# qgallouedec/deep_rl

Hardware: AMD Instinct MI355X
Metric: env-steps/sec + updates/sec, PPO CartPole-v1 4096 envs/GPU (higher is better)
Workload: dtype f32

## Files before the change

### deep_rl_amd/csrc/mi_grad_kernel.inc

```
struct __attribute__((aligned(16))) GV(grad_weights) {
#if GRAD_BX
    bf16x8 W2g[4 * 2 * 3 * 64];
    bf16x8 W2t[4 * 2 * 3 * 64];
#else
    float W2g[HID * HID];
    float W2t[HID * HID];
#endif
    float b1[HID], b2[HID];
    float W3[2 * HID];
    float W1s[HID * OBS];
    float b3s[4];
#if GRAD_BX
    union { unsigned short imgH[BX_IMG]; float bufB[TROWS * W2S]; } hb[GRAD_WAVES];
    unsigned short imgZ[GRAD_WAVES][BX_IMG];
    float xs[GRAD_WAVES][TROWS * 4];
#else
    float bufA[GRAD_WAVES][TROWS * W2S];
    float bufB[GRAD_WAVES][TROWS * W2S];
    float bufC[GRAD_WAVES][TROWS * W2S];
#endif
};
struct __attribute__((aligned(16))) GV(grad_smem) {
    union {
        GV(grad_weights) w;
        float red[GRAD_WAVES][RED_STRIDE];
    };
    double nrm[4];
    double nparts[256];
};
#if GRAD_BX
#define XS(row, k) xs[(row) * 4 + (k)]
#else
#define XS(row, k) bufA[(row) * W2S + HID + (k)]
#endif

template <bool ACTOR>
__device__ __forceinline__ void GV(grad_body)(GV(grad_smem)& sm, const float* __restrict__ params, const grad_pending_t& pend,
                                          const float* __restrict__ observations,
                                          const int64_t* __restrict__ actions, const float* __restrict__ log_probs,
                                          const float* __restrict__ advantages, const float* __restrict__ returns,
                                          const float* __restrict__ values, const int32_t* __restrict__ idx, int mb,
                                          const double* __restrict__ adv_sums, float clip_coef, float ent_coef, float vf_coef,
                                          float invn, float* __restrict__ part, unsigned vb, grad_role_t rl) {
    constexpr int NOUT = ACTOR ? 2 : 1;
    constexpr int BASE = ACTOR ? 0 : C_BASE;
    constexpr bool ANTI = ACTOR;
    constexpr int NHEAD = ANTI ? 1 : NOUT;
    const int tid = threadIdx.x, lane = tid & 63, wib = tid >> 6;
    const int j = lane & 15, g = lane >> 4;
    const bool pending = pend.grads != nullptr;
    const float* p = (pending ? pend.p_in : params) + BASE;
    GV(grad_weights)& W = sm.w;
#ifdef GRAD_STAMPS
    unsigned long long rt_in, rt_ready, rt_loop;
    asm volatile("s_memrealtime %0\n\ts_waitcnt lgkmcnt(0)" : "=s"(rt_in) :: "memory");
#endif

#ifdef GRAD_STAMPS
    unsigned long long pro_t[6] = {0, 0, 0, 0, 0, 0};
    asm volatile("s_memtime %0\n\ts_waitcnt lgkmcnt(0)" : "=s"(pro_t[0]) :: "memory");
#endif
    {
        const int q = (tid >> 4) & 15, cg = tid & 15;
        const bool writer = pending && rl.ri == 0;
        const bool w2t = tid < 256;
        constexpr int NT_A = N_W2, NT_B = HID + NOUT * HID;
        const bool has0 = tid < NT_A + NT_B, has1 = tid < NOUT;
        const int f0 = !has0 ? 0 : (tid < NT_A ? tid : N_B2 + (tid - NT_A));
        const int f1 = N_W3 + NOUT * HID + (has1 ? tid : 0);
        f32x4 w[4];
#pragma unroll
        for (int e = 0; e < 4; ++e) w[e] = w2t ? reinterpret_cast<const f32x4*>(p + N_W2)[(4 * q + e) * 16 + cg] : f32x4{0.0f, 0.0f, 0.0f, 0.0f};
        float sp0 = p[f0], sp1 = p[f1];
        if (pending) {
            f32x4 gg[4], mm[4], vv[4];
#pragma unroll
            for (int e = 0; e < 4; ++e) {
                const int at = w2t ? (4 * q + e) * 16 + cg : 0;
                gg[e] = reinterpret_cast<const f32x4*>(pend.grads + BASE + N_W2)[at];
                mm[e] = reinterpret_cast<const f32x4*>(pend.m_in + BASE + N_W2)[at];
                vv[e] = reinterpret_cast<const f32x4*>(pend.v_in + BASE + N_W2)[at];
            }
            const float sg0 = pend.grads[BASE + f0], sg1 = pend.grads[BASE + f1];
            float sm0 = pend.m_in[BASE + f0], sv0 = pend.v_in[BASE + f0], sm1 = pend.m_in[BASE + f1], sv1 = pend.v_in[BASE + f1];
            const bool hold = __hip_atomic_load(pend.gate, __ATOMIC_RELAXED, __HIP_MEMORY_SCOPE_AGENT) != 0u;
            const float a_w1 = hold ? 0.0f : pend.w1, a_b2 = hold ? 1.0f : pend.b2, a_w2 = hold ? 0.0f : pend.w2, a_ss = hold ? 0.0f : pend.step_size;
#ifdef GRAD_STAMPS
            asm volatile("s_memtime %0\n\ts_waitcnt lgkmcnt(0)" : "=s"(pro_t[1]) :: "memory");
#endif
            const float total = block_grad_norm(pend.grads, pend.norm_parts, NPARAMS, sm.nrm, sm.nparts);
#ifdef GRAD_STAMPS
            asm volatile("s_memtime %0\n\ts_waitcnt lgkmcnt(0)" : "=s"(pro_t[2]) :: "memory");
#endif
            float coef = pend.max_norm / (total + 1e-6f);
            coef = coef > 1.0f ? 1.0f : coef;
            if (pend.grad_norm && vb == 0 && tid == 0) *pend.grad_norm = total;
            if (w2t) {
#pragma unroll
                for (int e = 0; e < 4; ++e) {
#pragma unroll
                    for (int x = 0; x < 4; ++x) {
// ... 37 lines not shown
                unsigned h0, m0, l0, h1_, m1, l1;
                split3(w[0][x], w[1][x], h0, m0, l0); split3(w[2][x], w[3][x], h1_, m1, l1);
                const int lane_a = (i & 15) + 16 * (q & 3), slot = 4 * ((q >> 2) & 1);
                const int base = (((i >> 4) * 2 + (q >> 3)) * 3) * 64 * 8 + lane_a * 8 + slot;
                *reinterpret_cast<uint2*>(timg + base) = make_uint2(h0, h1_);
                *reinterpret_cast<uint2*>(timg + base + 64 * 8) = make_uint2(m0, m1);
                *reinterpret_cast<uint2*>(timg + base + 2 * 64 * 8) = make_uint2(l0, l1);
            }
#else
#pragma unroll
            for (int e = 0; e < 4; ++e) *reinterpret_cast<f32x4*>(&W.W2g[(cg * 64 + 4 * q + e) * 4]) = w[e] * GRAD_PS;
#pragma unroll
            for (int x = 0; x < 4; ++x) *reinterpret_cast<f32x4*>(&W.W2t[(q * 64 + 4 * cg + x) * 4]) = f32x4{w[0][x], w[1][x], w[2][x], w[3][x]};
#endif
        }
        if (has0) {
            if (tid < N_B1) W.W1s[tid] = GRAD_PS * sp0;
            else if (tid < NT_A) W.b1[tid - N_B1] = GRAD_PS * sp0;
            else if (tid < NT_A + HID) W.b2[tid - NT_A] = GRAD_PS * sp0;
            else W.W3[tid - NT_A - HID] = sp0;
        }
        if (has1) W.b3s[tid] = sp1;
    }

    float adv_mean = 0.0f, adv_rden = 1.0f;
    if constexpr (ACTOR) {
        const double s1 = adv_sums[0], s2 = adv_sums[1], cnt = adv_sums[2];
        const double mean = s1 / cnt;
        double var = (s2 - s1 * mean) / (cnt - 1.0);
        var = var < 0.0 ? 0.0 : var;
        adv_mean = (float)mean;
        adv_rden = 1.0f / ((float)sqrt(var) + 1e-8f);
    }

    const int n_tiles = (mb + TROWS - 1) / TROWS;
    const int half = rl.nr * 4;
    const bool split_ok = (gridDim.x % (2u << GRAD_ROLE_BIT)) == 0;
    const bool young = split_ok && wib >= 4;
    const int wi_half = rl.ri * 4 + (wib & 3);
    int tile, stride, tile_end;
    if (split_ok) {
        const int rounds = (n_tiles + half - 1) / half;
        const int old_rounds = (rounds * GRAD_OLD_SHARE + 8) / 16;
        const int split = old_rounds * half < n_tiles ? old_rounds * half : n_tiles;
        const int wi = wi_half;
        stride = half;
        tile = young ? split + wi : wi;
        tile_end = young ? n_tiles : split;
    } else {
        stride = rl.nr * GRAD_WAVES;
        tile = rl.ri * GRAD_WAVES + wib;
        tile_end = n_tiles;
    }
    auto tile_rid = [&](int t) { const int row = t * TROWS + j; return idx[row < mb ? row : mb - 1]; };
    int rid_next = tile_rid(tile + stride);
    row_in cur = gather_row<ACTOR>(tile_rid(tile), g, observations, actions, log_probs, advantages, returns, values);
#ifdef GRAD_STAMPS
    asm volatile("s_memtime %0\n\ts_waitcnt lgkmcnt(0)" : "=s"(pro_t[4]) :: "memory");
#endif
    __syncthreads();
    float w1f[4], b3[NOUT];
#pragma unroll
    for (int mt = 0; mt < 4; ++mt) w1f[mt] = W.W1s[4 * (16 * mt + j) + g];
#pragma unroll
    for (int a = 0; a < NOUT; ++a) b3[a] = W.b3s[a];
    f32x4 w3d[4];
    if constexpr (ANTI) {
#pragma unroll
        for (int mt = 0; mt < 4; ++mt) {
            const float4 w0 = *reinterpret_cast<const float4*>(&W.W3[16 * mt + 4 * g]), w1 = *reinterpret_cast<const float4*>(&W.W3[HID + 16 * mt + 4 * g]);
            w3d[mt] = f32x4{w0.x - w1.x, w0.y - w1.y, w0.z - w1.z, w0.w - w1.w};
        }
    }
#ifdef GRAD_STAMPS
    asm volatile("s_memtime %0\n\ts_waitcnt lgkmcnt(0)" : "=s"(pro_t[5]) :: "memory");
#endif

#if GRAD_BX
    f32x16 dW2x[2][2];
#pragma unroll
    for (int ot = 0; ot < 2; ++ot)
#pragma unroll
        for (int it2 = 0; it2 < 2; ++it2)
#pragma unroll
            for (int q = 0; q < 16; ++q) dW2x[ot][it2][q] = 0.0f;
    f32x4 db2v[4];
#pragma unroll
    for (int mt = 0; mt < 4; ++mt) db2v[mt] = f32x4{0.0f, 0.0f, 0.0f, 0.0f};
#else
    f32x4 dW2[4][4];
#pragma unroll
    for (int mo = 0; mo < 4; ++mo)
#pragma unroll
        for (int mi = 0; mi < 4; ++mi) dW2[mo][mi] = f32x4{0.0f, 0.0f, 0.0f, 0.0f};
#endif
    f32x4 dW1a = {0.0f, 0.0f, 0.0f, 0.0f}, dW1b = dW1a;
    f32x4 dW3v[NHEAD][4];
#pragma unroll
    for (int a = 0; a < NHEAD; ++a)
#pragma unroll
        for (int mt = 0; mt < 4; ++mt) dW3v[a][mt] = f32x4{0.0f, 0.0f, 0.0f, 0.0f};
    float db1 = 0.0f, db3[2] = {0.0f, 0.0f};
#if !GRAD_BX
    float db2[4] = {0.0f, 0.0f, 0.0f, 0.0f};
#endif
    float loss_a = 0.0f, loss_b = 0.0f;

#if GRAD_BX
    unsigned short* imgH = W.hb[wib].imgH;
    unsigned short* imgZ = W.imgZ[wib];
    float* bufB = W.hb[wib].bufB;
    float* xs = W.xs[wib];
#else
    float* bufA = W.bufA[wib];
    float* bufB = W.bufB[wib];
    float* bufC = W.bufC[wib];
#endif

#ifdef GRAD_STAMPS
    asm volatile("s_memrealtime %0\n\ts_waitcnt lgkmcnt(0)" : "=s"(rt_ready) :: "memory");
    unsigned long long stamp_acc[12] = {0, 0, 0, 0, 0, 0, 0, 0, 0, 0, 0, 0}, stamp_last, stamp_t0;
    asm volatile("s_memtime %0\n\ts_waitcnt lgkmcnt(0)" : "=s"(stamp_last) :: "memory");
    stamp_t0 = stamp_last;
#endif
    int it = 0;
    for (; tile < tile_end; tile += stride, ++it) {
        const bool valid = tile * TROWS + j < mb;
        const row_in nxt = gather_row<ACTOR>(rid_next, g, observations, actions, log_probs, advantages, returns, values);
        rid_next = tile_rid(tile + 2 * stride);

        XS(j, g) = cur.x;
        STAMP(0);

        f32x4 h1[4];
#pragma unroll
        for (int mt = 0; mt < 4; ++mt) {
            const float4 b = *reinterpret_cast<const float4*>(&W.b1[16 * mt + 4 * g]);
            h1[mt] = mfma16(w1f[mt], cur.x, f32x4{b.x, b.y, b.z, b.w});
        }
#pragma unroll
        for (int mt = 0; mt < 4; ++mt)
#pragma unroll
            for (int r = 0; r < 4; ++r) h1[mt][r] = GRAD_TANH(h1[mt][r]);
#if !GRAD_BX
#pragma unroll
        for (int mt = 0; mt < 4; ++mt) *reinterpret_cast<float4*>(bufA + j * W2S + 16 * mt + 4 * g) = make_float4(h1[mt][0], h1[mt][1], h1[mt][2], h1[mt][3]);
#endif
        STAMP(1);

        f32x4 h2[4];
#pragma unroll
        for (int mt = 0; mt < 4; ++mt) {
            const float4 b = *reinterpret_cast<const float4*>(&W.b2[16 * mt + 4 * g]);
            h2[mt] = f32x4{b.x, b.y, b.z, b.w};
        }
#if GRAD_BX
        wave_lds_fence();
#pragma unroll
        for (int sh = 0; sh < 2; ++sh) {
            const bx_parts bq = split8(h1[2 * sh], h1[2 * sh + 1]);
            bx_store_image(imgH, bq, sh, g, j);
#pragma unroll
            for (int mt = 0; mt < 4; ++mt) {
                bf16x8 a[3];
#pragma unroll
                for (int pp = 0; pp < 3; ++pp) a[pp] = W.W2g[((mt * 2 + sh) * 3 + pp) * 64 + lane];
                h2[mt] = bx_mac(a, bq, h2[mt]);
            }
        }
#else
#pragma unroll
        for (int c = 0; c < 4; ++c) {
            f32x4 a[4];
#pragma unroll
            for (int mt = 0; mt < 4; ++mt) a[mt] = *reinterpret_cast<const f32x4*>(&W.W2g[((4 * c + g) * 64 + 16 * mt + j) * 4]);
#pragma unroll
            for (int r = 0; r < 4; ++r)
#pragma unroll
                for (int mt = 0; mt < 4; ++mt) h2[mt] = mfma16(a[mt][r], h1[c][r], h2[mt]);
        }
#endif
        STAMP(2);
#pragma unroll
        for (int mt = 0; mt < 4; ++mt)
// ... 111 lines not shown
        for (int sh = 0; sh < 2; ++sh) {
            const bx_parts bq = split8(dz2[2 * sh], dz2[2 * sh + 1]);
            bx_store_image(imgZ, bq, sh, g, j);
#pragma unroll
            for (int mt = 0; mt < 4; ++mt) {
                bf16x8 a[3];
#pragma unroll
                for (int pp = 0; pp < 3; ++pp) a[pp] = W.W2t[((mt * 2 + sh) * 3 + pp) * 64 + lane];
                dz1[mt] = bx_mac(a, bq, dz1[mt]);
            }
        }
#pragma unroll
        for (int mt = 0; mt < 4; ++mt) db2v[mt] += dz2[mt];
        wave_lds_fence();
        {
            const int at = (lane >> 5) * BX_HALF + (lane & 31) * 8;
#pragma unroll
            for (int it2 = 0; it2 < 2; ++it2) {
                bf16x8 hbv[3];
#pragma unroll
                for (int pp = 0; pp < 3; ++pp) hbv[pp] = *reinterpret_cast<const bf16x8*>(imgH + pp * BX_PART + 32 * it2 * 8 + at);
#pragma unroll
                for (int ot = 0; ot < 2; ++ot) {
                    bf16x8 za[3];
#pragma unroll
                    for (int pp = 0; pp < 3; ++pp) za[pp] = *reinterpret_cast<const bf16x8*>(imgZ + pp * BX_PART + 32 * ot * 8 + at);
                    dW2x[ot][it2] = bx_mac32(za, hbv, dW2x[ot][it2]);
                }
            }
        }
#else
#pragma unroll
        for (int c = 0; c < 4; ++c) {
            f32x4 a[4];
#pragma unroll
            for (int mt = 0; mt < 4; ++mt) a[mt] = *reinterpret_cast<const f32x4*>(&W.W2t[((4 * c + g) * 64 + 16 * mt + j) * 4]);
#pragma unroll
            for (int r = 0; r < 4; ++r)
#pragma unroll
                for (int mt = 0; mt < 4; ++mt) dz1[mt] = mfma16(a[mt][r], dz2[c][r], dz1[mt]);
        }
#endif
#pragma unroll
        for (int mt = 0; mt < 4; ++mt)
#pragma unroll
            for (int r = 0; r < 4; ++r) { const float t = h1[mt][r]; dz1[mt][r] = dz1[mt][r] * __builtin_fmaf(-t, t, 1.0f); }

        STAMP(7);
        wave_lds_fence();
#pragma unroll
        for (int mt = 0; mt < 4; ++mt)
            *reinterpret_cast<float4*>(bufB + j * W2S + 16 * mt + 4 * g) = make_float4(dz1[mt][0], dz1[mt][1], dz1[mt][2], dz1[mt][3]);
        wave_lds_fence();
#pragma unroll
        for (int rr = 0; rr < TROWS; rr += 2) {
            const float z0 = bufB[rr * W2S + lane], z1v = bufB[(rr + 1) * W2S + lane];
            db1 += z0 + z1v;
            dW1a = mfma4(z0, XS(rr, lane & 3), dW1a);
            dW1b = mfma4(z1v, XS(rr + 1, lane & 3), dW1b);
        }

        STAMP(8);
#if !GRAD_BX
        wave_lds_fence();
#pragma unroll
        for (int s = 0; s < 4; ++s) {
            const int ro = (s + 4 * g) * W2S + j;
            float a[4], b[4];
#pragma unroll
            for (int m = 0; m < 4; ++m) { a[m] = bufC[ro + 16 * m]; b[m] = bufA[ro + 16 * m]; db2[m] += a[m]; }
#pragma unroll
            for (int mo = 0; mo < 4; ++mo)
#pragma unroll
                for (int mi = 0; mi < 4; ++mi) dW2[mo][mi] = mfma16(a[mo], b[mi], dW2[mo][mi]);
        }
#endif
        STAMP(9);
        cur = nxt;
        STAMP(10);
    }
#ifdef GRAD_STAMPS
    if (lane == 0) {
        unsigned long long* dbg = STAMP_BASE(part) + 32 * wib;
        unsigned long long now;
        asm volatile("s_memtime %0\n\ts_waitcnt lgkmcnt(0)" : "=s"(now) :: "memory");
        for (int k = 0; k < 11; ++k) dbg[k] = stamp_acc[k];
        dbg[11] = now - stamp_t0;
        dbg[12] = (unsigned long long)it;
        for (int k = 0; k < 6; ++k) dbg[20 + k] = pro_t[k];
    }
    asm volatile("s_memrealtime %0\n\ts_waitcnt lgkmcnt(0)" : "=s"(rt_loop) :: "memory");
#endif
    const f32x4 dW1 = dW1a + dW1b;

    __syncthreads();
    {
        float* slot = sm.red[wib];
#if GRAD_BX
#pragma unroll
        for (int ot = 0; ot < 2; ++ot)
#pragma unroll
            for (int it2 = 0; it2 < 2; ++it2)
#pragma unroll
                for (int qq = 0; qq < 4; ++qq) {
                    const int o = 32 * ot + 8 * qq + 4 * (lane >> 5), i = 32 * it2 + (lane & 31);
                    const f32x16& d = dW2x[ot][it2];
                    *reinterpret_cast<f32x4*>(&slot[((4 * (o >> 4) + (i >> 4)) * 64 + (i & 15) + 16 * ((o & 15) >> 2)) * 4]) =
                        f32x4{d[4 * qq], d[4 * qq + 1], d[4 * qq + 2], d[4 * qq + 3]};
                }
#else
#pragma unroll
        for (int mo = 0; mo < 4; ++mo)
#pragma unroll
            for (int mi = 0; mi < 4; ++mi) *reinterpret_cast<f32x4*>(&slot[((4 * mo + mi) * 64 + lane) * 4]) = dW2[mo][mi];
#endif
        float* sm_small = slot + HID * HID;
#pragma unroll
        for (int i = 0; i < 4; ++i) sm_small[(4 * (lane >> 2) + i) * 4 + (lane & 3)] = dW1[i];
        sm_small[256 + lane] = db1;
#if GRAD_BX
#pragma unroll
        for (int mt = 0; mt < 4; ++mt)
#pragma unroll
            for (int r = 0; r < 4; ++r) {
                float t = db2v[mt][r];
                t += dpp_xor1(t); t += dpp_xor2(t); t += dpp_half_mirror(t); t += dpp_mirror(t);
                if (j == 0) sm_small[320 + 16 * mt + 4 * g + r] = t;
            }
#else
#pragma unroll
        for (int m = 0; m < 4; ++m) {
            const float t = groups_sum(db2[m]);
// ... 26 lines not shown
    for (int k = 0; k < HID * HID / 4 / (64 * GRAD_WAVES); ++k) {
        const int i = tid + 64 * GRAD_WAVES * k;
        const f32x4 a0 = reinterpret_cast<const f32x4*>(sm.red[0])[i], a1 = reinterpret_cast<const f32x4*>(sm.red[1])[i];
        const f32x4 a2 = reinterpret_cast<const f32x4*>(sm.red[2])[i], a3 = reinterpret_cast<const f32x4*>(sm.red[3])[i];
        const f32x4 a4 = reinterpret_cast<const f32x4*>(sm.red[4])[i], a5 = reinterpret_cast<const f32x4*>(sm.red[5])[i];
        const f32x4 a6 = reinterpret_cast<const f32x4*>(sm.red[6])[i], a7 = reinterpret_cast<const f32x4*>(sm.red[7])[i];
        reinterpret_cast<f32x4*>(part + N_W2)[i] = ((a0 + a2) + (a1 + a3)) + ((a4 + a6) + (a5 + a7));
    }
    constexpr int N_SMALL = 384 + NOUT * HID + NOUT;
    for (int i = tid; i < 522; i += 64 * GRAD_WAVES) {
        if (i >= N_SMALL && i < 520) continue;
        float t = (sm.red[0][HID * HID + i] + sm.red[1][HID * HID + i]) + (sm.red[2][HID * HID + i] + sm.red[3][HID * HID + i]);
        t += (sm.red[4][HID * HID + i] + sm.red[5][HID * HID + i]) + (sm.red[6][HID * HID + i] + sm.red[7][HID * HID + i]);
        int dst;
        if (i < 256) dst = N_W1 + i;
        else if (i < 320) dst = N_B1 + (i - 256);
        else if (i < 384) dst = N_B2 + (i - 320);
        else if (i < N_SMALL) dst = N_W3 + (i - 384);
        else dst = PART_LOSS + (i - 520);
        part[dst] = t;
    }
#ifdef GRAD_STAMPS
    if (lane == 0) {
        unsigned long long rt_out;
        asm volatile("s_memrealtime %0\n\ts_waitcnt lgkmcnt(0)" : "=s"(rt_out) :: "memory");
        unsigned long long* dbg = STAMP_BASE(part) + 32 * wib;
        dbg[13] = rt_in; dbg[14] = rt_ready; dbg[15] = rt_loop; dbg[16] = rt_out;
        const unsigned hw_id = __builtin_amdgcn_s_getreg((31 << 11) | 4), xcc = __builtin_amdgcn_s_getreg((31 << 11) | 20);
        dbg[17] = ((unsigned long long)xcc << 32) | hw_id;
    }
#endif
}

__global__ void __launch_bounds__(64 * GRAD_WAVES, GRAD_WPS)
GV(grad_kernel)(const float* __restrict__ params, grad_pending_t pend, const float* __restrict__ observations, const int64_t* __restrict__ actions,
            const float* __restrict__ log_probs, const float* __restrict__ advantages, const float* __restrict__ returns,
            const float* __restrict__ values, const int32_t* __restrict__ idx, int mb, const double* __restrict__ adv_sums,
            float clip_coef, float ent_coef, float vf_coef, float invn, float* __restrict__ workspace) {
    __shared__ GV(grad_smem) sm;
    MI_INSIDE_SCOPE(MI_PROF_GRAD);
    const unsigned rb = GRAD_ROLE_BIT;
    const unsigned lowmask = (1u << rb) - 1u;
    const unsigned vb = (gridDim.x & ((2u << rb) - 1u)) ? blockIdx.x
                                                        : ((blockIdx.x >> rb) & 1u) | (((blockIdx.x & lowmask) | ((blockIdx.x >> (rb + 1)) << rb)) << 1);
    float* part = workspace + (size_t)vb * PART_STRIDE;
    const grad_role_t rl = grad_role(vb, (int)gridDim.x);
    if (rl.role == 0)
        GV(grad_body)<true>(sm, params, pend, observations, actions, log_probs, advantages, returns, values, idx, mb, adv_sums, clip_coef,
                        ent_coef, vf_coef, invn, part, vb, rl);
    else
        GV(grad_body)<false>(sm, params, pend, observations, actions, log_probs, advantages, returns, values, idx, mb, adv_sums, clip_coef,
                         ent_coef, vf_coef, invn, part, vb, rl);
}

#undef XS
```

### deep_rl_amd/csrc/mi_update.hip

```cpp
#include "mi_common.h"

typedef float f32x16 __attribute__((ext_vector_type(16)));
typedef float f32x4 __attribute__((ext_vector_type(4)));

__global__ void __launch_bounds__(64) gae_kernel(const float* __restrict__ rewards, const float* __restrict__ dones,
                                                 const float* __restrict__ values, int T, int N, float gamma, float lam,
                                                 float* __restrict__ adv, float* __restrict__ returns) {
    const int i = blockIdx.x * blockDim.x + threadIdx.x;
    if (i >= N) return;
    float last = 0.0f;
    float vnext = values[(size_t)T * N + i];
    adv[(size_t)T * N + i] = 0.0f;
    returns[(size_t)T * N + i] = 0.0f + vnext;
#pragma unroll 8
    for (int t = T - 1; t >= 0; --t) {
        const size_t c = (size_t)t * N + i, n = c + N;
        const float vcur = values[c];
        const float a = gamma * (1.0f - dones[n]);
        const float b = vnext + lam * last;
        float v = rewards[n] + a * b;
        v = v - vcur;
        adv[c] = v;
        returns[c] = v + vcur;
        last = v;
// ... 258 lines not shown
        }
        if ((lane & 15) == 0) {
            const int row = lane >> 4, k0 = (row & 1) + 9 * (row >> 1);
#pragma unroll
            for (int q = 0; q < 4; ++q) sparts[w + 8 * (2 * q + k0)] = s[q];
            if ((row & 1) == 0) sparts[w + 8 * (8 + 9 * (row >> 1))] = s[4];
        }
        __syncthreads();
        if (t < 256) S = sparts[t];
    } else {
        const bool perm = n == NPARAMS;
        if (t < 256) sparts[t] = 0.0;
        __syncthreads();
        constexpr int U = 6;
        for (int b0 = w; b0 < nb; b0 += nw * U) {
            float x[U];
#pragma unroll
            for (int u = 0; u < U; ++u) {
                const int b = b0 + nw * u, p = 64 * b + lane;
                x[u] = (b < nb && p < n) ? grads[perm ? ppo_slab_to_param(p) : p] : 0.0f;
            }
#pragma unroll
            for (int u = 0; u < U; ++u) {
                const int b = b0 + nw * u;
                const double sb = wave_butterfly_f64((double)x[u] * (double)x[u]);
                if (lane == 0 && b < nb) sparts[b & 255] = sparts[b & 255] + sb;
            }
        }
        __syncthreads();
        if (t < 256) S = sparts[t];
    }
    S = wave_butterfly_f64(S);
    if (t < 256 && lane == 0) ws[w] = S;
    __syncthreads();
    return (float)sqrt((ws[0] + ws[1]) + (ws[2] + ws[3]));
}

struct grad_pending_t {
    const float* grads;
    const float* p_in; const float* m_in; const float* v_in;
    float* p_out; float* m_out; float* v_out;
    float* grad_norm;
    const double* norm_parts;
    const uint32_t* gate;
    float w1, b2, w2, step_size, rbc2, eps, max_norm;
};

struct grad_role_t { int role, ri, nr; };
__host__ __device__ inline grad_role_t grad_role(unsigned vb, int n_blocks) {
    return grad_role_t{(int)(vb & 1u), (int)(vb >> 1), n_blocks >> 1};
}
__host__ __device__ inline int grad_slab(int role, int ri) { return 2 * ri + role; }

struct row_in {
    float x;
    int act;
    float f0, f1;
};

template <bool ACTOR>
__device__ __forceinline__ row_in gather_row(int rid, int g, const float* __restrict__ observations, const int64_t* __restrict__ actions,
                                             const float* __restrict__ log_probs, const float* __restrict__ advantages,
                                             const float* __restrict__ returns, const float* __restrict__ values) {
    row_in r;
    r.x = observations[4 * (size_t)rid + g];
    if constexpr (ACTOR) {
        r.act = reinterpret_cast<const int*>(actions)[2 * (size_t)rid];
        r.f0 = log_probs[rid]; r.f1 = advantages[rid];
    } else {
        r.act = 0;
        r.f0 = returns[rid]; r.f1 = values[rid];
    }
    return r;
}

#ifdef GRAD_STAMPS
#define STAMP(k) do { __builtin_amdgcn_sched_barrier(0); { unsigned long long t_; asm volatile("s_memtime %0\n\ts_waitcnt lgkmcnt(0)" : "=s"(t_) :: "memory"); \
                      stamp_acc[k] += t_ - stamp_last; stamp_last = t_; } __builtin_amdgcn_sched_barrier(0); } while (0)
#define STAMP_BASE(part) (reinterpret_cast<unsigned long long*>((part) + (size_t)(GRAD_MAX_BLOCKS / 2) * PART_STRIDE))
#else
#define STAMP(k) do {} while (0)
#endif

#define GRAD_BX 0
#define GV(x) x##_f32
#include "mi_grad_kernel.inc"
#undef GRAD_BX
#undef GV
#define GRAD_BX 1
#define GV(x) x##_bx
#include "mi_grad_kernel.inc"
#undef GRAD_BX
#undef GV

#define RED_PARAMS 64
#define RED_GROUPS 16
template <int WORLD>
__global__ void __launch_bounds__(RED_PARAMS * RED_GROUPS)
grad_reduce_kernel(const float* __restrict__ workspace, int n_blocks, float ent_coef, float vf_coef, double inv_count,
                   float* __restrict__ grads, float* __restrict__ loss_terms, double* __restrict__ norm_parts, const p2p_args_t x) {
    MI_INSIDE_SCOPE(MI_PROF_REDUCE);
    const int pblocks = (NPARAMS + RED_PARAMS - 1) / RED_PARAMS;
    if ((int)blockIdx.x < pblocks) {
        __shared__ float part[RED_GROUPS][RED_PARAMS];
        const int pl = threadIdx.x & (RED_PARAMS - 1), sg = threadIdx.x >> 6;
        const int p = blockIdx.x * RED_PARAMS + pl;
        float acc = 0.0f;
        const int role = p < C_BASE ? 0 : 1;
        const int off = p - (role ? C_BASE : 0);
        if (p < NPARAMS) {
            const float* src = workspace + off;
            const int nr = n_blocks >> 1;
            if (nr <= 9 * RED_GROUPS) {
                float v[9];
#pragma unroll
                for (int u = 0; u < 9; ++u) { const int k = sg + RED_GROUPS * u; v[u] = k < nr ? src[(size_t)grad_slab(role, k) * PART_STRIDE] : 0.0f; }
#pragma unroll
                for (int u = 0; u < 9; ++u) if (sg + RED_GROUPS * u < nr) acc += v[u];
            } else {
#pragma unroll 4
                for (int k = sg; k < nr; k += RED_GROUPS) acc += src[(size_t)grad_slab(role, k) * PART_STRIDE];
            }
        }
        part[sg][pl] = acc;
// ... 97 lines not shown
                           const float* advantages, const float* returns, const float* values, const int32_t* idx, int mb, const double* adv_sums,
                           float clip_coef, float ent_coef, float vf_coef, double inv_count, void* workspace, float* grads, float* loss_terms,
                           hipStream_t s, void* p2p = nullptr) {
    int blocks = grad_blocks();
    const int tiles = (mb + TROWS - 1) / TROWS;
    const int need = 2 * ((tiles + GRAD_WAVES - 1) / GRAD_WAVES);
    if (need < blocks) blocks = need;
    {
        mi_prof_scope prof(MI_PROF_GRAD, s);
        if (g_contraction == MI_CONTRACTION_BF16X3)
            grad_kernel_bx<<<blocks, 64 * GRAD_WAVES, 0, s>>>(params, pend, observations, actions, log_probs, advantages, returns, values, idx, mb,
                                                              adv_sums, clip_coef, ent_coef, vf_coef, (float)inv_count, (float*)workspace);
        else
            grad_kernel_f32<<<blocks, 64 * GRAD_WAVES, 0, s>>>(params, pend, observations, actions, log_probs, advantages, returns, values, idx, mb,
                                                               adv_sums, clip_coef, ent_coef, vf_coef, (float)inv_count, (float*)workspace);
    }
    MI_LAUNCH_CHECK();
    {
        mi_prof_scope prof(MI_PROF_REDUCE, s);
        static_assert((NPARAMS + RED_PARAMS - 1) / RED_PARAMS == NORM_BLOCKS && RED_PARAMS == 64, "one norm block per reduction workgroup");
        p2p_args_t x;
        memset(&x, 0, sizeof(x));
        int world = 0;
        if (p2p) {
            if (loss_terms != grads + NPARAMS) { mi_set_error("ppo_grad_launch: the P2P exchange needs loss_terms == grads + MI_PPO_NPARAMS"); return MI_EINVAL; }
            int rc = mi_comm_p2p_next(p2p, (size_t)NPARAMS + 4, &x, &world, s);
            if (rc) return rc;
        }
        const float* ws = (const float*)workspace;
        double* np = ws_norm_parts(workspace);
        switch (world) {
            case 0: grad_reduce_launch<0>(s, ws, blocks, ent_coef, vf_coef, inv_count, grads, loss_terms, np, x); break;
            case 1: grad_reduce_launch<1>(s, ws, blocks, ent_coef, vf_coef, inv_count, grads, loss_terms, np, x); break;
            case 2: grad_reduce_launch<2>(s, ws, blocks, ent_coef, vf_coef, inv_count, grads, loss_terms, np, x); break;
            case 3: grad_reduce_launch<3>(s, ws, blocks, ent_coef, vf_coef, inv_count, grads, loss_terms, np, x); break;
            case 4: grad_reduce_launch<4>(s, ws, blocks, ent_coef, vf_coef, inv_count, grads, loss_terms, np, x); break;
            case 5: grad_reduce_launch<5>(s, ws, blocks, ent_coef, vf_coef, inv_count, grads, loss_terms, np, x); break;
            case 6: grad_reduce_launch<6>(s, ws, blocks, ent_coef, vf_coef, inv_count, grads, loss_terms, np, x); break;
            case 7: grad_reduce_launch<7>(s, ws, blocks, ent_coef, vf_coef, inv_count, grads, loss_terms, np, x); break;
            default: grad_reduce_launch<8>(s, ws, blocks, ent_coef, vf_coef, inv_count, grads, loss_terms, np, x); break;
        }
    }
    MI_LAUNCH_CHECK();
    return MI_OK;
}

extern "C" int mi_ppo_minibatch_grad(const float* params, const float* observations, const int64_t* actions,
                                     const float* log_probs, const float* advantages, const float* returns,
                                     const float* values, const int32_t* idx, int mb, const double* adv_sums, float clip_coef,
                                     float ent_coef, float vf_coef, double inv_count, void* workspace, float* grads,
                                     float* loss_terms, void* stream) {
    MI_CHECK_ARG(params && observations && actions && log_probs && advantages && returns && values && idx && adv_sums, "NULL input");
    MI_CHECK_ARG(workspace && grads, "NULL workspace/grads");
    MI_CHECK_ARG(mb > 0, "mb must be positive");
    return ppo_grad_launch(params, no_pending(), observations, actions, log_probs, advantages, returns, values, idx, mb, adv_sums, clip_coef, ent_coef,
                           vf_coef, inv_count, workspace, grads, loss_terms, (hipStream_t)stream);
}

__global__ void __launch_bounds__(512) clip_adam_kernel(const float* p_in, const float* m_in, const float* v_in, float* p_out, float* m_out, float* v_out,
                                                         const float* __restrict__ grads, int n, float w1, float b2,
                                                         float w2, float step_size, float rbc2, float eps, float max_norm,
                                                         float* __restrict__ grad_norm, const double* __restrict__ norm_parts, const uint32_t* __restrict__ gate) {
    __shared__ double ws[4], sparts[256];
    MI_INSIDE_SCOPE(MI_PROF_CLIP_ADAM);
    const bool hold = mi_gate_closed(gate);
    const int i = blockIdx.x * blockDim.x + threadIdx.x;
    const bool live = i < n;
    float pm = live ? m_in[i] : 0.0f, pv = live ? v_in[i] : 0.0f;
    const float pp = live ? p_in[i] : 0.0f, pg = live ? grads[i] : 0.0f;
    const float total = block_grad_norm(grads, norm_parts, n, ws, sparts);
    float coef = max_norm / (total + 1e-6f);
    coef = coef > 1.0f ? 1.0f : coef;
    if (grad_norm && blockIdx.x == 0 && threadIdx.x == 0) *grad_norm = total;
    if (live) {
        float np = pp;
        if (!hold) np = mi_adam_elem(pp, pg * coef, pm, pv, w1, b2, w2, step_size, rbc2, eps);
        m_out[i] = pm; v_out[i] = pv;
        p_out[i] = np;
    }
}

struct adam_consts_t { float w1, b2, w2, step_size, rbc2, eps; };
static adam_consts_t adam_consts(int64_t step, double lr, double beta1, double beta2, double eps) {
    const double bc1 = 1.0 - pow(beta1, (double)step), bc2 = 1.0 - pow(beta2, (double)step);
    adam_consts_t k;
    k.w1 = (float)(1.0 - beta1); k.b2 = (float)beta2; k.w2 = (float)(1.0 - beta2);
    k.step_size = (float)(lr / bc1); k.rbc2 = (float)(1.0 / sqrt(bc2)); k.eps = (float)eps;
    return k;
}

static int clip_adam_launch(const float* p_in, const float* m_in, const float* v_in, float* p_out, float* m_out, float* v_out, const float* grads, int n,
                            const adam_consts_t& k, float max_norm, float* grad_norm, const double* norm_parts, hipStream_t s, const uint32_t* gate = nullptr) {
    mi_prof_scope prof(MI_PROF_CLIP_ADAM, s);
    const int threads = n == NPARAMS ? 512 : 256;
    clip_adam_kernel<<<(n + threads - 1) / threads, threads, 0, s>>>(p_in, m_in, v_in, p_out, m_out, v_out, grads, n, k.w1, k.b2, k.w2, k.step_size, k.rbc2, k.eps, max_norm,
                                                                    grad_norm, norm_parts, gate);
    MI_LAUNCH_CHECK();
    return MI_OK;
}

int mi_clip_adam_gated(float* params, const float* grads, float* exp_avg, float* exp_avg_sq, int n, int64_t step, double lr, double beta1, double beta2, double eps,
                       float max_norm, float* grad_norm, void* comm, void* stream) {
    return clip_adam_launch(params, exp_avg, exp_avg_sq, params, exp_avg, exp_avg_sq, grads, n, adam_consts(step, lr, beta1, beta2, eps), max_norm, grad_norm,
                            nullptr, (hipStream_t)stream, mi_comm_gate(comm));
}

extern "C" int mi_clip_adam(float* params, const float* grads, float* exp_avg, float* exp_avg_sq, int n, int64_t step, double lr,
                            double beta1, double beta2, double eps, float max_norm, float* grad_norm, void* stream) {
// ... 70 lines not shown
    hipStream_t s = (hipStream_t)stream;
    const int mb = n_rows / n_minibatch;
    if (mb % PS_PER_BLOCK == 0 && epochs <= PS_MAX_EPOCHS) {
        MI_HIP(hipMemsetAsync(sums_all, 0, sizeof(double) * 3 * (size_t)n_minibatch * epochs, s));
        ps_epochs_t pe;
        for (int ep = 0; ep < epochs; ++ep) {
            const uint64_t key = mi_perm_key(seed, (uint64_t)update_index, (uint64_t)ep);
            pe.k0[ep] = (uint32_t)key; pe.k1[ep] = (uint32_t)(key >> 32); pe.out[ep] = perm_all + (size_t)ep * n_rows;
        }
        uint32_t bits = 1;
        while ((1u << bits) < (uint32_t)n_rows) ++bits;
        if (bits < 2) bits = 2;
        mi_prof_scope prof(MI_PROF_STATS, s);
        perm_stats_kernel<<<dim3((n_rows + PS_PER_BLOCK - 1) / PS_PER_BLOCK, epochs), 256, 0, s>>>((uint32_t)n_rows, bits / 2, bits - bits / 2, pe, mb, n_minibatch, advantages,
                                                                                                 sums_all);
        MI_LAUNCH_CHECK();
        return MI_OK;
    }
    for (int ep = 0; ep < epochs; ++ep) {
        int rc = mi_make_perm((uint32_t)n_rows, mi_perm_key(seed, (uint64_t)update_index, (uint64_t)ep), perm_all + (size_t)ep * n_rows, stream);
        if (rc) return rc;
        rc = mi_adv_stats(advantages, perm_all + (size_t)ep * n_rows, mb, n_minibatch, sums_all + (size_t)3 * n_minibatch * ep, stream);
        if (rc) return rc;
    }
    return MI_OK;
}

struct opt_set_t { float* p; float* m; float* v; };

static int ppo_update_impl(void* handle, const mi_ppo_buffers_t* b, const mi_ppo_hparams_t* hp, void* comm, int world, void* stream);

extern "C" int mi_ppo_update(void* handle, const mi_ppo_buffers_t* b, const mi_ppo_hparams_t* hp, void* stream) {
    return ppo_update_impl(handle, b, hp, nullptr, 1, stream);
}

extern "C" int mi_ppo_update_sharded(void* handle, const mi_ppo_buffers_t* b, const mi_ppo_hparams_t* hp, void* comm, void* stream) {
    int world = 1;
    if (comm) {
        int rc = mi_comm_poll_impl(comm);
        if (rc) return rc;
        rc = mi_comm_info(comm, &world, nullptr, nullptr, nullptr);
        if (rc) return rc;
        MI_CHECK_ARG(b && b->loss_terms == b->grads + NPARAMS, "sharded update: loss_terms must be grads + MI_PPO_NPARAMS (one buffer, one all-reduce)");
    }
    return ppo_update_impl(handle, b, hp, comm, world, stream);
}

static int ppo_update_impl(void* handle, const mi_ppo_buffers_t* b, const mi_ppo_hparams_t* hp, void* comm, int world, void* stream) {
    MI_CHECK_ARG(handle && b && hp, "NULL pointer");
    MI_CHECK_ARG(hp->T > 0 && hp->n_minibatch > 0 && hp->update_epochs > 0, "bad hyper-parameters");
    mi_env* e = (mi_env*)handle;
    const int N = e->n, B = hp->T * N;
    MI_CHECK_ARG(B % hp->n_minibatch == 0, "T*N must be divisible by n_minibatch");
    const int mb = B / hp->n_minibatch;
    const bool fused = (mb % PS_PER_BLOCK) == 0;
    const bool p2p = comm != nullptr && mi_comm_p2p_fused_ok(comm);
    const bool sharded_norm = (world > 1 && !p2p) || g_assume_sharded != 0;
    int rc = mi_rollout_gae_internal(handle, b->params, hp->T, b->obs_cur, b->observations, b->values, b->actions, b->log_probs, b->rewards,
                                     b->dones, b->episodes, b->episode_stats, b->max_ep, hp->gamma, hp->gae_lambda, b->advantages, b->returns,
                                     fused ? b->adv_sums : nullptr, 3 * hp->n_minibatch * hp->update_epochs, b->episode_stats_next, stream);
    if (rc) return rc;
    hipStream_t s = (hipStream_t)stream;
    if (fused && hp->update_epochs <= PS_MAX_EPOCHS) {
        ps_epochs_t pe;
        for (int ep = 0; ep < hp->update_epochs; ++ep) {
            const uint64_t key = mi_perm_key(e->seed, (uint64_t)hp->update_index, (uint64_t)ep);
            pe.k0[ep] = (uint32_t)key; pe.k1[ep] = (uint32_t)(key >> 32); pe.out[ep] = b->perm + (size_t)ep * B;
        }
        uint32_t bits = 1;
        while ((1u << bits) < (uint32_t)B) ++bits;
        if (bits < 2) bits = 2;
        mi_prof_scope prof(MI_PROF_STATS, s);
        perm_stats_kernel<<<dim3((B + PS_PER_BLOCK - 1) / PS_PER_BLOCK, hp->update_epochs), 256, 0, s>>>((uint32_t)B, bits / 2, bits - bits / 2, pe, mb, hp->n_minibatch,
                                                                                                       b->advantages, b->adv_sums);
        MI_LAUNCH_CHECK();
    } else {
        rc = mi_ppo_perms_and_stats(e->seed, hp->update_index, hp->update_epochs, B, hp->n_minibatch, b->advantages, b->perm, b->adv_sums, stream);
        if (rc) return rc;
    }
    if (comm) {
        mi_prof_scope prof(MI_PROF_COMM_STATS, s);
        rc = mi_comm_allreduce_impl(comm, b->adv_sums, (size_t)3 * hp->n_minibatch * hp->update_epochs, 1, s);
        if (rc) return rc;
    }
    float* spare = reinterpret_cast<float*>(b->workspace) + (size_t)(GRAD_MAX_BLOCKS - GRAD_SPARE_SLABS) * PART_STRIDE;
    const opt_set_t caller = {b->params, b->exp_avg, b->exp_avg_sq};
    const opt_set_t sets[2] = {{spare, spare + STATE_STRIDE, spare + 2 * STATE_STRIDE},
                               {spare + 3 * STATE_STRIDE, spare + 4 * STATE_STRIDE, spare + 5 * STATE_STRIDE}};
    opt_set_t cur = caller;
    int64_t step = hp->opt_step;
    bool owed = false;
    int flip = 0;
    for (int ep = 0; ep < hp->update_epochs; ++ep) {
        const double* sums = b->adv_sums + (size_t)3 * hp->n_minibatch * ep;
        const int32_t* perm = b->perm + (size_t)ep * B;
        for (int k = 0; k < hp->n_minibatch; ++k) {
            grad_pending_t pend = no_pending();
            if (owed) {
                const adam_consts_t c = adam_consts(step, hp->lr, hp->beta1, hp->beta2, hp->eps);
                const opt_set_t out = sets[flip];
                flip ^= 1;
                pend.grads = b->grads; pend.p_in = cur.p; pend.m_in = cur.m; pend.v_in = cur.v; pend.p_out = out.p; pend.m_out = out.m; pend.v_out = out.v;
                pend.grad_norm = b->grad_norm; pend.w1 = c.w1; pend.b2 = c.b2; pend.w2 = c.w2; pend.step_size = c.step_size; pend.rbc2 = c.rbc2; pend.eps = c.eps;
                pend.max_norm = hp->max_grad_norm;
                pend.norm_parts = sharded_norm ? nullptr : ws_norm_parts(b->workspace);
                pend.gate = ppo_gate(comm);
// ... 209 lines not shown
```

Measured before the change: 396.3 million.

## Split grad loop into full and ragged tiles, use 32-bit gathers and LDS bases

Restructures the gradient kernel's tile loop so that full tiles run without bounds clamping and at most one ragged tail tile runs separately. Global gathers now use 32-bit byte offsets with scalar bases instead of 64-bit indexing, and the wave index is made uniform via readfirstlane. Per-wave LDS buffers are regrouped into one struct, LDS read pointers are hoisted out of the loop, and the x values are read back as vector loads. The aim is less address arithmetic and fewer VGPRs in the hot loop, paid for by a new 2^28-row limit on storage and extra code size.

```diff
diff --git a/deep_rl_amd/csrc/mi_grad_kernel.inc b/deep_rl_amd/csrc/mi_grad_kernel.inc
--- a/deep_rl_amd/csrc/mi_grad_kernel.inc
+++ b/deep_rl_amd/csrc/mi_grad_kernel.inc
@@ -10,16 +10,19 @@
     float W3[2 * HID];
     float W1s[HID * OBS];
     float b3s[4];
-#if GRAD_BX
-    union { unsigned short imgH[BX_IMG]; float bufB[TROWS * W2S]; } hb[GRAD_WAVES];
-    unsigned short imgZ[GRAD_WAVES][BX_IMG];
-    float xs[GRAD_WAVES][TROWS * 4];
-#else
-    float bufA[GRAD_WAVES][TROWS * W2S];
-    float bufB[GRAD_WAVES][TROWS * W2S];
-    float bufC[GRAD_WAVES][TROWS * W2S];
-#endif
+    struct {
+#if GRAD_BX
+        union { unsigned short imgH[BX_IMG]; float bufB[TROWS * W2S]; } hb;
+        unsigned short imgZ[BX_IMG];
+#else
+        float bufA[TROWS * W2S];
+        float bufB[TROWS * W2S];
+        float bufC[TROWS * W2S];
+#endif
+        float xs[4 * TROWS];
+    } __attribute__((aligned(16))) st[GRAD_WAVES];
 };
+static_assert(TROWS == 16, "xs is read back as four b128 per lane");
 struct __attribute__((aligned(16))) GV(grad_smem) {
     union {
         GV(grad_weights) w;
@@ -28,11 +31,6 @@
     double nrm[4];
     double nparts[256];
 };
-#if GRAD_BX
-#define XS(row, k) xs[(row) * 4 + (k)]
-#else
-#define XS(row, k) bufA[(row) * W2S + HID + (k)]
-#endif
 
 template <bool ACTOR>
 __device__ __forceinline__ void GV(grad_body)(GV(grad_smem)& sm, const float* __restrict__ params, const grad_pending_t& pend,
@@ -46,7 +44,8 @@
     constexpr int BASE = ACTOR ? 0 : C_BASE;
     constexpr bool ANTI = ACTOR;
     constexpr int NHEAD = ANTI ? 1 : NOUT;
-    const int tid = threadIdx.x, lane = tid & 63, wib = tid >> 6;
+    const int tid = threadIdx.x, lane = tid & 63;
+    const int wib = __builtin_amdgcn_readfirstlane(tid >> 6);
     const int j = lane & 15, g = lane >> 4;
     const bool pending = pend.grads != nullptr;
     const float* p = (pending ? pend.p_in : params) + BASE;
@@ -190,9 +189,24 @@
         tile = rl.ri * GRAD_WAVES + wib;
         tile_end = n_tiles;
     }
+    const int full_tiles = mb / TROWS;
+    const int lim = tile_end < full_tiles ? tile_end : full_tiles;
+    unsigned j4 = 4u * (unsigned)j;
+    auto full_rid = [&](int t) {
+        const int tc = t < full_tiles ? t : full_tiles - 1;
+        gbl_bytes* base = (gbl_bytes*)(idx + (size_t)tc * TROWS);
+        asm volatile("" : "+s"(base), "+v"(j4));
+        return *(const __attribute__((address_space(1))) int*)(base + j4);
+    };
     auto tile_rid = [&](int t) { const int row = t * TROWS + j; return idx[row < mb ? row : mb - 1]; };
-    int rid_next = tile_rid(tile + stride);
-    row_in cur = gather_row<ACTOR>(tile_rid(tile), g, observations, actions, log_probs, advantages, returns, values);
+    int rid_next = 0;
+    row_in cur = {0.0f, 0, 0.0f, 0.0f}, nxt = cur;
+    if (tile < lim) {
+        rid_next = full_rid(tile + stride);
+        cur = gather_row<ACTOR>(full_rid(tile), g, observations, actions, log_probs, advantages, returns, values);
+    }
+    const bool only_ragged = tile >= lim && tile < tile_end;
+    if (only_ragged) cur = gather_row<ACTOR>(tile_rid(tile), g, observations, actions, log_probs, advantages, returns, values);
 #ifdef GRAD_STAMPS
     asm volatile("s_memtime %0\n\ts_waitcnt lgkmcnt(0)" : "=s"(pro_t[4]) :: "memory");
 #endif
@@ -245,14 +259,21 @@
     float loss_a = 0.0f, loss_b = 0.0f;
 
 #if GRAD_BX
-    unsigned short* imgH = W.hb[wib].imgH;
-    unsigned short* imgZ = W.imgZ[wib];
-    float* bufB = W.hb[wib].bufB;
-    float* xs = W.xs[wib];
-#else
-    float* bufA = W.bufA[wib];
-    float* bufB = W.bufB[wib];
-    float* bufC = W.bufC[wib];
+    unsigned short* imgH = W.st[wib].hb.imgH;
+    unsigned short* imgZ = W.st[wib].imgZ;
+    float* bufB = W.st[wib].hb.bufB;
+#else
+    float* bufA = W.st[wib].bufA;
+    float* bufB = W.st[wib].bufB;
+    float* bufC = W.st[wib].bufC;
+#endif
+    float* xs = W.st[wib].xs;
+    const lds_f32* rdB[TROWS / 4];
+#pragma unroll
+    for (int k = 0; k < TROWS / 4; ++k) rdB[k] = lds_read_base(bufB + 4 * k * W2S + lane);
+#if !GRAD_BX
+    const lds_f32* rdA = lds_read_base(bufA + 4 * g * W2S + j);
+    const lds_f32* rdC = lds_read_base(bufC + 4 * g * W2S + j);
 #endif
 
 #ifdef GRAD_STAMPS
@@ -261,13 +282,11 @@
     asm volatile("s_memtime %0\n\ts_waitcnt lgkmcnt(0)" : "=s"(stamp_last) :: "memory");
     stamp_t0 = stamp_last;
 #endif
-    int it = 0;
-    for (; tile < tile_end; tile += stride, ++it) {
-        const bool valid = tile * TROWS + j < mb;
-        const row_in nxt = gather_row<ACTOR>(rid_next, g, observations, actions, log_probs, advantages, returns, values);
-        rid_next = tile_rid(tile + 2 * stride);
-
-        XS(j, g) = cur.x;
+    [[maybe_unused]] int it = 0;
+    auto tile_body = [&](auto ragged, const int t, const row_in& cur) __attribute__((always_inline)) {
+        constexpr bool RAGGED = decltype(ragged)::value;
+        const bool valid = !RAGGED || t * TROWS + j < mb;
+        xs[TROWS * g + j] = cur.x;
         STAMP(0);
 
         f32x4 h1[4];
@@ -485,12 +504,15 @@
         for (int mt = 0; mt < 4; ++mt)
             *reinterpret_cast<float4*>(bufB + j * W2S + 16 * mt + 4 * g) = make_float4(dz1[mt][0], dz1[mt][1], dz1[mt][2], dz1[mt][3]);
         wave_lds_fence();
+        f32x4 xv[TROWS / 4];
+#pragma unroll
+        for (int q = 0; q < TROWS / 4; ++q) xv[q] = *reinterpret_cast<const f32x4*>(xs + TROWS * (lane & 3) + 4 * q);
 #pragma unroll
         for (int rr = 0; rr < TROWS; rr += 2) {
-            const float z0 = bufB[rr * W2S + lane], z1v = bufB[(rr + 1) * W2S + lane];
+            const float z0 = rdB[rr >> 2][(rr & 3) * W2S], z1v = rdB[(rr + 1) >> 2][((rr + 1) & 3) * W2S];
             db1 += z0 + z1v;
-            dW1a = mfma4(z0, XS(rr, lane & 3), dW1a);
-            dW1b = mfma4(z1v, XS(rr + 1, lane & 3), dW1b);
+            dW1a = mfma4(z0, xv[rr >> 2][rr & 3], dW1a);
+            dW1b = mfma4(z1v, xv[(rr + 1) >> 2][(rr + 1) & 3], dW1b);
         }
 
         STAMP(8);
@@ -498,10 +520,9 @@
         wave_lds_fence();
 #pragma unroll
         for (int s = 0; s < 4; ++s) {
-            const int ro = (s + 4 * g) * W2S + j;
             float a[4], b[4];
 #pragma unroll
-            for (int m = 0; m < 4; ++m) { a[m] = bufC[ro + 16 * m]; b[m] = bufA[ro + 16 * m]; db2[m] += a[m]; }
+            for (int m = 0; m < 4; ++m) { a[m] = rdC[s * W2S + 16 * m]; b[m] = rdA[s * W2S + 16 * m]; db2[m] += a[m]; }
 #pragma unroll
             for (int mo = 0; mo < 4; ++mo)
 #pragma unroll
@@ -509,8 +530,21 @@
         }
 #endif
         STAMP(9);
+    };
+    auto full_step = [&](const row_in& c, row_in& n, const int t) __attribute__((always_inline)) {
+        n = gather_row<ACTOR>(rid_next, g, observations, actions, log_probs, advantages, returns, values);
+        rid_next = full_rid(t + 2 * stride);
+        tile_body(grad_tag<false>{}, t, c);
+        ++it;
+    };
+    for (; tile < lim; tile += stride) {
+        full_step(cur, nxt, tile);
         cur = nxt;
-        STAMP(10);
+    }
+    if (tile < tile_end) {
+        if (!only_ragged) cur = gather_row<ACTOR>(tile_rid(tile), g, observations, actions, log_probs, advantages, returns, values);
+        tile_body(grad_tag<true>{}, tile, cur);
+        ++it;
     }
 #ifdef GRAD_STAMPS
     if (lane == 0) {
@@ -643,5 +677,3 @@
         GV(grad_body)<false>(sm, params, pend, observations, actions, log_probs, advantages, returns, values, idx, mb, adv_sums, clip_coef,
                          ent_coef, vf_coef, invn, part, vb, rl);
 }
-
-#undef XS
diff --git a/deep_rl_amd/csrc/mi_update.hip b/deep_rl_amd/csrc/mi_update.hip
--- a/deep_rl_amd/csrc/mi_update.hip
+++ b/deep_rl_amd/csrc/mi_update.hip
@@ -334,24 +334,39 @@
 }
 __host__ __device__ inline int grad_slab(int role, int ri) { return 2 * ri + role; }
 
+typedef __attribute__((address_space(3))) float lds_f32;
+typedef const __attribute__((address_space(1))) char gbl_bytes;
+__device__ __forceinline__ const lds_f32* lds_read_base(const float* p) {
+    const lds_f32* q = (const lds_f32*)p;
+    asm volatile("" : "+v"(q));
+    return q;
+}
+template <bool B> struct grad_tag{ static constexpr bool value = B; };
+
 struct row_in {
     float x;
     int act;
     float f0, f1;
 };
 
+#define GRAD_MAX_ROWS (1 << 28)
+template <typename T>
+__device__ __forceinline__ T load_at(const void* __restrict__ base, unsigned byte_off) {
+    return *reinterpret_cast<const T*>(reinterpret_cast<const char*>(base) + byte_off);
+}
 template <bool ACTOR>
 __device__ __forceinline__ row_in gather_row(int rid, int g, const float* __restrict__ observations, const int64_t* __restrict__ actions,
                                              const float* __restrict__ log_probs, const float* __restrict__ advantages,
                                              const float* __restrict__ returns, const float* __restrict__ values) {
     row_in r;
-    r.x = observations[4 * (size_t)rid + g];
+    const unsigned urid = (unsigned)rid;
+    r.x = load_at<float>(observations, 16u * urid + 4u * (unsigned)g);
     if constexpr (ACTOR) {
-        r.act = reinterpret_cast<const int*>(actions)[2 * (size_t)rid];
-        r.f0 = log_probs[rid]; r.f1 = advantages[rid];
+        r.act = load_at<int>(actions, 8u * urid);
+        r.f0 = load_at<float>(log_probs, 4u * urid); r.f1 = load_at<float>(advantages, 4u * urid);
     } else {
         r.act = 0;
-        r.f0 = returns[rid]; r.f1 = values[rid];
+        r.f0 = load_at<float>(returns, 4u * urid); r.f1 = load_at<float>(values, 4u * urid);
     }
     return r;
 }
@@ -555,8 +570,8 @@
                                      float* loss_terms, void* stream) {
     MI_CHECK_ARG(params && observations && actions && log_probs && advantages && returns && values && idx && adv_sums, "NULL input");
     MI_CHECK_ARG(workspace && grads, "NULL workspace/grads");
-    MI_CHECK_ARG(mb > 0, "mb must be positive");
-    return ppo_grad_launch(params, no_pending(), observations, actions, log_probs, advantages, returns, values, idx, mb, adv_sums, clip_coef, ent_coef,
+    MI_CHECK_ARG(mb > 0 && mb <= GRAD_MAX_ROWS, "mb must be positive and at most 2^28");
+    return ppo_grad_launch(params, no_pending(),observations, actions, log_probs, advantages, returns, values, idx, mb, adv_sums, clip_coef, ent_coef,
                            vf_coef, inv_count, workspace, grads, loss_terms, (hipStream_t)stream);
 }
 
@@ -733,6 +748,7 @@
     mi_env* e = (mi_env*)handle;
     const int N = e->n, B = hp->T * N;
     MI_CHECK_ARG(B % hp->n_minibatch == 0, "T*N must be divisible by n_minibatch");
+    MI_CHECK_ARG((long long)(hp->T + 1) * N <= GRAD_MAX_ROWS, "(T+1)*N exceeds 2^28 storage rows (the gradient kernel gathers with 32-bit byte offsets)");
     const int mb = B / hp->n_minibatch;
     const bool fused = (mb % PS_PER_BLOCK) == 0;
     const bool p2p = comm != nullptr && mi_comm_p2p_fused_ok(comm);
```

After: 401.3 million (median of 6 runs). 1.3% higher.
